# ESA-PRL/planning-path_planning

Hardware: NVIDIA B200
Metric: plans_per_s (higher is better)
Workload: dtype f64

## Files before the change

planning-path_planning_b200/build.py:

```python
import os
import subprocess
import sys

HERE = os.path.dirname(os.path.abspath(__file__))
ROOT = os.path.dirname(HERE)
INCLUDE = os.path.join(ROOT, "include")
BUILD = os.path.join(ROOT, "build")
CUDA_SO = os.path.join(HERE, "libdymu_cuda.so")
HOST_SO = os.path.join(HERE, "libdymu_b200.so")

NVCC = os.environ.get("DYMU_NVCC", "/usr/local/cuda/bin/nvcc")
CXX = os.environ.get("DYMU_CXX", "/usr/bin/g++")

NVCC_FLAGS = [
    "-gencode", "arch=compute_100a,code=sm_100a", "-lineinfo", "-O3", "-std=c++17",
    "-fmad=false", "-Xcompiler", "-fPIC", "-ccbin", CXX, "-I", INCLUDE,
]
CXX_FLAGS = ["-O2", "-std=c++14", "-fPIC", "-Wall", "-ffp-contract=off", "-I", INCLUDE,
             "-I", os.path.join(HERE, "src"), "-I", os.path.join(HERE, "shim")]


def _newer(target, sources):
    if not os.path.exists(target):
        return True
    t = os.path.getmtime(target)
    return any(os.path.getmtime(s) > t for s in sources)


def _run(cmd, verbose):
    if verbose:
        print(" ".join(cmd), flush=True)
    r = subprocess.run(cmd, stdout=subprocess.PIPE, stderr=subprocess.STDOUT, text=True)
    if r.returncode != 0:
        sys.stderr.write(r.stdout)
        raise RuntimeError("build step failed: " + " ".join(cmd[:3]) + " ...")
    if verbose and r.stdout:
        print(r.stdout)
    return r.stdout


def cuda_sources():
    d = os.path.join(HERE, "csrc")
    return sorted(os.path.join(d, f) for f in os.listdir(d) if f.endswith(".cu"))


def host_sources():
    d = os.path.join(HERE, "src")
    srcs = sorted(os.path.join(d, f) for f in os.listdir(d) if f.endswith(".cpp"))
    srcs.append(os.path.join(HERE, "capi", "planner_capi.cpp"))
    return srcs


def build_cuda(force=False, verbose=False, ptxas_v=False):
    os.makedirs(BUILD, exist_ok=True)
    headers = [os.path.join(HERE, "csrc", f) for f in os.listdir(os.path.join(HERE, "csrc"))
               if f.endswith((".cuh", ".h"))] + [os.path.join(INCLUDE, "dymu_cuda.h")]
    objs = []
    log = ""
    for src in cuda_sources():
        obj = os.path.join(BUILD, os.path.basename(src)[:-3] + ".o")
        objs.append(obj)
        if force or _newer(obj, [src] + headers):
            extra = ["-Xptxas", "-v"] if ptxas_v else []
            if os.environ.get("DYMU_FIM_PROFILE"):
                extra.append("-DDYMU_FIM_PROFILE")
            if os.environ.get("DYMU_LOCAL_PROFILE"):
                extra.append("-DDYMU_LOCAL_PROFILE")
            log += _run([NVCC] + NVCC_FLAGS + extra + ["-c", src, "-o", obj], verbose)
    if force or _newer(CUDA_SO, objs):
        _run([NVCC, "-shared", "-gencode", "arch=compute_100a,code=sm_100a", "-ccbin", CXX,
              "-o", CUDA_SO] + objs + ["-cudart", "shared"], verbose)
    return log


def build_host(force=False, verbose=False):
    srcs = host_sources()
    hdrs = [os.path.join(HERE, "src", f) for f in os.listdir(os.path.join(HERE, "src"))
            if f.endswith((".hpp", ".h"))]
    hdrs += [os.path.join(INCLUDE, f) for f in os.listdir(INCLUDE)]
    if force or _newer(HOST_SO, srcs + hdrs + [CUDA_SO]):
        _run([CXX] + CXX_FLAGS + ["-shared", "-DDYMU_CAPI_B200"] + srcs +
             ["-o", HOST_SO, "-L", HERE, "-ldymu_cuda", "-Wl,-rpath,$ORIGIN"], verbose)


def build_all(force=False, verbose=False, ptxas_v=False):
    log = build_cuda(force, verbose, ptxas_v)
    if os.path.exists(os.path.join(HERE, "src", "DyMu.hpp")):
        build_host(force, verbose)
    return log


if __name__ == "__main__":
    out = build_all(force="--force" in sys.argv, verbose="--verbose" in sys.argv,
                    ptxas_v="--ptxas" in sys.argv)
    if "--ptxas" in sys.argv:
        print(out)
    print("built", CUDA_SO, "and", HOST_SO if os.path.exists(HOST_SO) else "(host lib pending)")
```

planning-path_planning_b200/csrc/dymu_path.cu:

```cuda
#include <limits.h>

#include "dymu_ctx.cuh"

namespace
{
constexpr int PATCH = 64;
constexpr int PATCH_LEAD = 20;

struct Patch
{
    double* t;
    double* e;
    double* gx;
    double* gy;
    int x0, y0;
    bool valid;
};

struct PathArgs
{
    const double* T;
    const double* elev;
    uint32_t pitch, nx, ny;
    double gres, tau;
    double x0, y0;
    uint32_t goal_i, goal_j;
    double* out;
    uint32_t cap;
    uint32_t* result;
};

__device__ __forceinline__ double grad_axis(double f, bool has_lo, double flo, bool has_hi,
                                            double fhi)
{
    const double inf = DYMU_INF;
    if ((!has_lo && !has_hi) || (has_lo && has_hi && flo == inf && fhi == inf)) return 0;
    if (!has_lo || flo == inf)
    {
        if (!has_hi) return 0;
        return fhi - f;
    }
    if (!has_hi || fhi == inf) return f - flo;
    return (fhi - flo) * 0.5;
}

__device__ __forceinline__ void grad_node(const PathArgs& a, const Patch& pt, uint32_t i, uint32_t j,
                                          double& dnx, double& dny)
{
    const double* Tc = pt.t + ((int)j - pt.y0) * PATCH + ((int)i - pt.x0);
    double f = *Tc;
    bool hl = i > 0, hr = i + 1 < a.nx, hd = j > 0, hu = j + 1 < a.ny;
    double fl = hl ? Tc[-1] : 0, fr = hr ? Tc[1] : 0;
    double fd = hd ? Tc[-PATCH] : 0, fu = hu ? Tc[PATCH] : 0;
    double dx = grad_axis(f, hl, fl, hr, fr);
    double dy = grad_axis(f, hd, fd, hu, fu);
    if ((dx == 0) && (dy == 0))
    {
        dnx = 0;
        dny = 0;
    }
    else
    {
        double n = sqrt(dx * dx + dy * dy);
        dnx = dx / n;
        dny = dy / n;
    }
}

constexpr int PATH_THREADS = 256;

struct PatchCmd
{
    int x0, y0;
};

__device__ __forceinline__ void load_patch(const PathArgs& a, double* pt_t, double* pt_e, int x0, int y0)
{
    for (int k = threadIdx.x; k < PATCH * PATCH; k += PATH_THREADS)
    {
        int r = k / PATCH, c = k % PATCH;
        int gx = x0 + c, gy = y0 + r;
        double tv = DYMU_INF, ev = 0.0;
        if (gx >= 0 && gy >= 0 && gx < (int)a.nx && gy < (int)a.ny)
        {
            tv = __ldcg(a.T + (size_t)gy * a.pitch + gx);
            ev = a.elev[(size_t)gy * a.pitch + gx];
        }
        pt_t[k] = tv;
        pt_e[k] = ev;
    }
}

__device__ __forceinline__ void patch_gradients(const PathArgs& a, const Patch& pt)
{
    for (int k = threadIdx.x; k < PATCH * PATCH; k += PATH_THREADS)
    {
        int r = k / PATCH, c = k % PATCH;
        int gx = pt.x0 + c, gy = pt.y0 + r;
        double dnx = 0, dny = 0;
        if (r >= 1 && c >= 1 && r < PATCH - 1 && c < PATCH - 1 && gx >= 0 && gy >= 0 && gx < (int)a.nx
            && gy < (int)a.ny)
            grad_node(a, pt, (uint32_t)gx, (uint32_t)gy, dnx, dny);
        pt.gx[k] = dnx;
        pt.gy[k] = dny;
    }
}

__device__ __forceinline__ void ensure_patch(const PathArgs& a, Patch& pt, PatchCmd* cmd, int lane, int cx,
                                             int cy, double dirx, double diry)
{
    if (pt.valid && cx - 1 >= pt.x0 && cy - 1 >= pt.y0 && cx + 2 < pt.x0 + PATCH && cy + 2 < pt.y0 + PATCH)
        return;
    int lx = (dirx == dirx) ? (int)(dirx * PATCH_LEAD) : 0, ly = (diry == diry) ? (int)(diry * PATCH_LEAD) : 0;
    lx = max(-PATCH_LEAD, min(PATCH_LEAD, lx));
    ly = max(-PATCH_LEAD, min(PATCH_LEAD, ly));
    pt.x0 = cx - PATCH / 2 + lx;
    pt.y0 = cy - PATCH / 2 + ly;
    pt.valid = true;
    if (lane == 0)
    {
        cmd->x0 = pt.x0;
        cmd->y0 = pt.y0;
    }
    __syncthreads();
    load_patch(a, pt.t, pt.e, pt.x0, pt.y0);
    __syncthreads();
    patch_gradients(a, pt);
    __syncthreads();
}

template <bool UNIT_RES>
__device__ __forceinline__ bool next_waypoint(const PathArgs& a, Patch& pt, PatchCmd* cmd, int lane,
                                              double wx, double wy, double& z, double& dCx,
                                              double& dCy, double& nx_, double& ny_)
{
    double gx = UNIT_RES ? wx : wx / a.gres, gy = UNIT_RES ? wy : wy / a.gres;
    if (!(gx >= 0.0) || !(gy >= 0.0) || !(gx < (double)(a.nx - 1)) || !(gy < (double)(a.ny - 1)))
        return false;
    uint32_t cx = (uint32_t)gx, cy = (uint32_t)gy;
    double da = gx - (double)cx, db = gy - (double)cy;
    ensure_patch(a, pt, cmd, lane, (int)cx, (int)cy, -dCx, -dCy);
    const int k00 = ((int)cy - pt.y0) * PATCH + ((int)cx - pt.x0);
    const int k10 = k00 + 1, k01 = k00 + PATCH, k11 = k00 + PATCH + 1;
    const double gx00 = pt.gx[k00], gx10 = pt.gx[k10], gx01 = pt.gx[k01], gx11 = pt.gx[k11];
    const double gy00 = pt.gy[k00], gy10 = pt.gy[k10], gy01 = pt.gy[k01], gy11 = pt.gy[k11];
    const double e00 = pt.e[k00], e10 = pt.e[k10], e01 = pt.e[k01], e11 = pt.e[k11];
    dCx = dymu_interp(da, db, gx00, gx01, gx10, gx11);
    dCy = dymu_interp(da, db, gy00, gy01, gy10, gy11);
    z = dymu_interp(da, db, e00, e10, e01, e11);
    nx_ = wx - a.gres * a.tau * dCx;
    ny_ = wy - a.gres * a.tau * dCy;
    return true;
}

__device__ __forceinline__ double dist2(double ax, double ay, double bx, double by)
{
    return (ax - bx) * (ax - bx) + (ay - by) * (ay - by);
}
__device__ __forceinline__ double next_up(double x) { return __longlong_as_double(__double_as_longlong(x) + 1); }
__device__ __forceinline__ double next_down(double x) { return __longlong_as_double(__double_as_longlong(x) - 1); }
__device__ double sqrt_gt_threshold(double c)
{
    if (!(c > 0)) return (c == 0) ? 0.0 : -1.0;
    double t = c * c;
    while (sqrt(t) > c) t = next_down(t);
    while (sqrt(next_up(t)) <= c) t = next_up(t);
    return t;
}
__device__ double sqrt_lt_threshold(double c)
{
    if (!(c > 0)) return 0.0;
    double t = c * c;
    while (sqrt(t) < c) t = next_up(t);
    while (t > 0 && sqrt(next_down(t)) >= c) t = next_down(t);
    return t;
}

template <bool UNIT_RES>
__global__ void __launch_bounds__(PATH_THREADS, 1) k_global_path(const PathArgs* args_arr)
{
    const PathArgs a = args_arr[blockIdx.x];
    const int lane = threadIdx.x & 31;
    extern __shared__ __align__(16) double path_smem[];
    __shared__ PatchCmd cmd;
    Patch pt;
    pt.t = path_smem;
    pt.e = path_smem + PATCH * PATCH;
    pt.gx = path_smem + 2 * PATCH * PATCH;
    pt.gy = path_smem + 3 * PATCH * PATCH;
    pt.x0 = pt.y0 = 0;
    pt.valid = false;
    if (threadIdx.x >= 32)
    {
        for (;;)
        {
            __syncthreads();
            const int x0 = cmd.x0, y0 = cmd.y0;
            if (x0 == INT_MIN) return;
            pt.x0 = x0;
            pt.y0 = y0;
            load_patch(a, pt.t, pt.e, x0, y0);
            __syncthreads();
            patch_gradients(a, pt);
            __syncthreads();
        }
    }
    const double sx = a.gres * (double)a.goal_i, sy = a.gres * (double)a.goal_j;
    uint32_t n = 0, status = DYMU_PATH_OK;
    double wx = a.x0, wy = a.y0, z, dCx = 0, dCy = 0, nx_, ny_;

    auto push = [&](double x, double y, double zz, double dx, double dy) -> bool {
        if (n >= a.cap) return false;
        if (lane == 0)
        {
            double* o = a.out + (size_t)5 * n;
            o[0] = x; o[1] = y; o[2] = zz; o[3] = dx; o[4] = dy;
        }
        n++;
        return true;
    };

    if (!next_waypoint<UNIT_RES>(a, pt, &cmd, lane, wx, wy, z, dCx, dCy, nx_, ny_)) status = DYMU_PATH_OUTSIDE;
    else if (isnan(nx_) || isnan(ny_)) status = DYMU_PATH_NAN;
    else
    {
        push(wx, wy, z, dCx, dCy);
        wx = nx_;
        wy = ny_;
        const double far2 = sqrt_gt_threshold(2.0 * a.gres);
        const double stall2 = sqrt_lt_threshold(0.01 * a.tau * a.gres);
        while (dist2(wx, wy, sx, sy) > far2)
        {
            if (!next_waypoint<UNIT_RES>(a, pt, &cmd, lane, wx, wy, z, dCx, dCy, nx_, ny_))
            {
                status = DYMU_PATH_OUTSIDE;
                break;
            }
            if (!push(wx, wy, z, dCx, dCy))
            {
                status = DYMU_PATH_CAPACITY;
                break;
            }
            if (dist2(wx, wy, nx_, ny_) < stall2)
            {
                status = DYMU_PATH_STALLED;
                break;
            }
            wx = nx_;
            wy = ny_;
        }
    }
    if (lane == 0)
    {
        a.result[0] = n;
        a.result[1] = status;
        cmd.x0 = INT_MIN;
    }
    __syncthreads();
}

int launch_paths(dymu_ctx* ctx, uint32_t n, size_t smem, const PathArgs* d_args)
{
    auto kernel = (ctx->gres == 1.0) ? k_global_path<true> : k_global_path<false>;
    DYMU_CUDA_TRY(ctx, cudaFuncSetAttribute(kernel, cudaFuncAttributeMaxDynamicSharedMemorySize, (int)smem));
    kernel<<<n, PATH_THREADS, smem, ctx->stream>>>(d_args);
    return DYMU_OK;
}
}

extern "C" {

int dymu_extract_global_path(dymu_ctx* ctx, uint32_t slot, double x0, double y0, double tau,
                             uint32_t goal_i, uint32_t goal_j, double* out, uint32_t cap,
                             uint32_t* n_out, int* status)
{
    DYMU_GUARD(ctx);
    if (!ctx || !out || !n_out || !status || cap == 0 || slot >= ctx->n_slots) return DYMU_ERR_ARG;
    if (goal_i >= ctx->nx || goal_j >= ctx->ny) return DYMU_ERR_ARG;
    size_t out_bytes = (size_t)cap * 5 * sizeof(double);
    size_t hdr = 256;
    DYMU_TRY(dymu_internal_scratch(ctx, hdr + out_bytes, hdr + out_bytes));
    PathArgs* h_args = (PathArgs*)ctx->h_pinned;
    PathArgs a;
    a.T = ctx->T + (size_t)slot * ctx->pitch * ctx->rows;
    a.elev = ctx->elev;
    a.pitch = ctx->pitch; a.nx = ctx->nx; a.ny = ctx->ny;
    a.gres = ctx->gres; a.tau = tau; a.x0 = x0; a.y0 = y0;
    a.goal_i = goal_i; a.goal_j = goal_j;
    a.out = (double*)((char*)ctx->d_scratch + hdr);
    a.cap = cap;
    a.result = (uint32_t*)((char*)ctx->d_scratch + sizeof(PathArgs));
    static_assert(sizeof(PathArgs) + 8 <= 256, "path header overflow");
    *h_args = a;
    DYMU_CUDA_TRY(ctx, cudaMemcpyAsync(ctx->d_scratch, h_args, sizeof(PathArgs),
                                       cudaMemcpyHostToDevice, ctx->stream));
    const size_t smem = 4 * PATCH * PATCH * sizeof(double);
    DYMU_TRY(launch_paths(ctx, 1, smem, (const PathArgs*)ctx->d_scratch));
    ctx->launches++;
    DYMU_CUDA_TRY(ctx, cudaGetLastError());
    uint32_t* h_res = (uint32_t*)((char*)ctx->h_pinned + sizeof(PathArgs));
    DYMU_CUDA_TRY(ctx, cudaMemcpyAsync(h_res, a.result, 8, cudaMemcpyDeviceToHost, ctx->stream));
    DYMU_CUDA_TRY(ctx, cudaStreamSynchronize(ctx->stream));
    *n_out = h_res[0];
    *status = (int)h_res[1];
    if (h_res[0])
    {
        DYMU_CUDA_TRY(ctx, cudaMemcpyAsync(out, a.out, (size_t)h_res[0] * 5 * sizeof(double),
                                           cudaMemcpyDeviceToHost, ctx->stream));
        DYMU_CUDA_TRY(ctx, cudaStreamSynchronize(ctx->stream));
    }
    return DYMU_OK;
}

int dymu_extract_global_path_batch(dymu_ctx* ctx, uint32_t n, const uint32_t* slots,
                                   const double* xy0, double tau, const uint32_t* goal_ij,
                                   double* out, uint32_t cap, uint32_t* n_out, int* status)
{
    DYMU_GUARD(ctx);
    if (!ctx || !slots || !xy0 || !goal_ij || !out || !n_out || !status || n == 0 || cap == 0)
        return DYMU_ERR_ARG;
    for (uint32_t q = 0; q < n; ++q)
        if (slots[q] >= ctx->n_slots || goal_ij[2 * q] >= ctx->nx || goal_ij[2 * q + 1] >= ctx->ny)
            return DYMU_ERR_ARG;
    const size_t hdr = (((size_t)n * (sizeof(PathArgs) + 8)) + 255) & ~(size_t)255;
    const size_t out_bytes = (size_t)n * cap * 5 * sizeof(double);
    DYMU_TRY(dymu_internal_scratch(ctx, hdr + out_bytes, hdr));
    PathArgs* h_args = (PathArgs*)ctx->h_pinned;
    char* d_base = (char*)ctx->d_scratch;
    uint32_t* d_res = (uint32_t*)(d_base + (size_t)n * sizeof(PathArgs));
    for (uint32_t q = 0; q < n; ++q)
    {
        PathArgs a;
        a.T = ctx->T + (size_t)slots[q] * ctx->pitch * ctx->rows;
        a.elev = ctx->elev;
        a.pitch = ctx->pitch; a.nx = ctx->nx; a.ny = ctx->ny;
        a.gres = ctx->gres; a.tau = tau; a.x0 = xy0[2 * q]; a.y0 = xy0[2 * q + 1];
        a.goal_i = goal_ij[2 * q]; a.goal_j = goal_ij[2 * q + 1];
        a.out = (double*)(d_base + hdr) + (size_t)q * cap * 5;
        a.cap = cap;
        a.result = d_res + 2 * q;
        h_args[q] = a;
    }
    DYMU_CUDA_TRY(ctx, cudaMemcpyAsync(d_base, h_args, (size_t)n * sizeof(PathArgs), cudaMemcpyHostToDevice,
                                       ctx->stream));
    const size_t smem = 4 * PATCH * PATCH * sizeof(double);
    DYMU_TRY(launch_paths(ctx, n, smem, (const PathArgs*)d_base));
    ctx->launches++;
    DYMU_CUDA_TRY(ctx, cudaGetLastError());
    uint32_t* h_res = (uint32_t*)((char*)ctx->h_pinned + (size_t)n * sizeof(PathArgs));
    DYMU_CUDA_TRY(ctx, cudaMemcpyAsync(h_res, d_res, (size_t)n * 8, cudaMemcpyDeviceToHost, ctx->stream));
    DYMU_CUDA_TRY(ctx, cudaStreamSynchronize(ctx->stream));
    for (uint32_t q = 0; q < n; ++q)
    {
        n_out[q] = h_res[2 * q];
        status[q] = (int)h_res[2 * q + 1];
        if (n_out[q])
            DYMU_CUDA_TRY(ctx, cudaMemcpyAsync(out + (size_t)q * cap * 5,
                                               (double*)(d_base + hdr) + (size_t)q * cap * 5,
                                               (size_t)n_out[q] * 5 * sizeof(double), cudaMemcpyDeviceToHost,
                                               ctx->stream));
    }
    DYMU_CUDA_TRY(ctx, cudaStreamSynchronize(ctx->stream));
    return DYMU_OK;
}

}
```

Before: 99.37.

## Double-buffer prefetched gradient windows with warp-specialized helper threads in path kernel

Restructures the path-extraction kernel so one warp walks the gradient descent while the other warps build the next 64x64 window (gradients plus elevation) into a second shared-memory buffer, coordinated through named barriers. It predicts where the walk will leave the current window and prefetches there, so window building is meant to overlap with walking instead of stalling it. Gradients are now computed straight from global T, which drops the staging pass and the extra block-wide syncs. The walk step also uses clamped window indexing with an in-window flag in place of a per-step bounds check. The cost is more complex synchronization: a wrong prediction still forces a blocking rebuild, and a shutdown path with a stop flag is needed. It also adds an optional profiling build flag.

```diff
diff --git a/planning-path_planning_b200/build.py b/planning-path_planning_b200/build.py
--- a/planning-path_planning_b200/build.py
+++ b/planning-path_planning_b200/build.py
@@ -66,6 +66,8 @@
                 extra.append("-DDYMU_FIM_PROFILE")
             if os.environ.get("DYMU_LOCAL_PROFILE"):
                 extra.append("-DDYMU_LOCAL_PROFILE")
+            if os.environ.get("DYMU_PATH_PROFILE"):
+                extra.append("-DDYMU_PATH_PROFILE")
             log += _run([NVCC] + NVCC_FLAGS + extra + ["-c", src, "-o", obj], verbose)
     if force or _newer(CUDA_SO, objs):
         _run([NVCC, "-shared", "-gencode", "arch=compute_100a,code=sm_100a", "-ccbin", CXX,
diff --git a/planning-path_planning_b200/csrc/dymu_path.cu b/planning-path_planning_b200/csrc/dymu_path.cu
--- a/planning-path_planning_b200/csrc/dymu_path.cu
+++ b/planning-path_planning_b200/csrc/dymu_path.cu
@@ -1,21 +1,20 @@
 #include <limits.h>
+#include <stdio.h>
+#include <stdlib.h>
 
 #include "dymu_ctx.cuh"
 
 namespace
 {
 constexpr int PATCH = 64;
+constexpr int P2 = PATCH * PATCH;
+constexpr int WIN_DOUBLES = 3 * P2;
+constexpr size_t PATH_SMEM = 2 * WIN_DOUBLES * sizeof(double);
 constexpr int PATCH_LEAD = 20;
-
-struct Patch
-{
-    double* t;
-    double* e;
-    double* gx;
-    double* gy;
-    int x0, y0;
-    bool valid;
-};
+constexpr int PATH_THREADS = 256;
+constexpr int HELPERS = PATH_THREADS - 32;
+constexpr int BUILD_BATCH = 4;
+constexpr int BAR_CMD = 1, BAR_DONE = 2;
 
 struct PathArgs
 {
@@ -28,6 +27,9 @@
     double* out;
     uint32_t cap;
     uint32_t* result;
+#ifdef DYMU_PATH_PROFILE
+    unsigned long long* prof;
+#endif
 };
 
 __device__ __forceinline__ double grad_axis(double f, bool has_lo, double flo, bool has_hi,
@@ -44,113 +46,139 @@
     return (fhi - flo) * 0.5;
 }
 
-__device__ __forceinline__ void grad_node(const PathArgs& a, const Patch& pt, uint32_t i, uint32_t j,
-                                          double& dnx, double& dny)
-{
-    const double* Tc = pt.t + ((int)j - pt.y0) * PATCH + ((int)i - pt.x0);
-    double f = *Tc;
-    bool hl = i > 0, hr = i + 1 < a.nx, hd = j > 0, hu = j + 1 < a.ny;
-    double fl = hl ? Tc[-1] : 0, fr = hr ? Tc[1] : 0;
-    double fd = hd ? Tc[-PATCH] : 0, fu = hu ? Tc[PATCH] : 0;
-    double dx = grad_axis(f, hl, fl, hr, fr);
-    double dy = grad_axis(f, hd, fd, hu, fu);
-    if ((dx == 0) && (dy == 0))
-    {
-        dnx = 0;
-        dny = 0;
-    }
-    else
-    {
-        double n = sqrt(dx * dx + dy * dy);
-        dnx = dx / n;
-        dny = dy / n;
-    }
-}
-
-constexpr int PATH_THREADS = 256;
-
-struct PatchCmd
-{
-    int x0, y0;
+struct WinCmd
+{
+    int x0, y0, buf, stop;
 };
 
-__device__ __forceinline__ void load_patch(const PathArgs& a, double* pt_t, double* pt_e, int x0, int y0)
-{
-    for (int k = threadIdx.x; k < PATCH * PATCH; k += PATH_THREADS)
-    {
-        int r = k / PATCH, c = k % PATCH;
-        int gx = x0 + c, gy = y0 + r;
-        double tv = DYMU_INF, ev = 0.0;
-        if (gx >= 0 && gy >= 0 && gx < (int)a.nx && gy < (int)a.ny)
-        {
-            tv = __ldcg(a.T + (size_t)gy * a.pitch + gx);
-            ev = a.elev[(size_t)gy * a.pitch + gx];
-        }
-        pt_t[k] = tv;
-        pt_e[k] = ev;
-    }
-}
-
-__device__ __forceinline__ void patch_gradients(const PathArgs& a, const Patch& pt)
-{
-    for (int k = threadIdx.x; k < PATCH * PATCH; k += PATH_THREADS)
-    {
-        int r = k / PATCH, c = k % PATCH;
-        int gx = pt.x0 + c, gy = pt.y0 + r;
-        double dnx = 0, dny = 0;
-        if (r >= 1 && c >= 1 && r < PATCH - 1 && c < PATCH - 1 && gx >= 0 && gy >= 0 && gx < (int)a.nx
-            && gy < (int)a.ny)
-            grad_node(a, pt, (uint32_t)gx, (uint32_t)gy, dnx, dny);
-        pt.gx[k] = dnx;
-        pt.gy[k] = dny;
-    }
-}
-
-__device__ __forceinline__ void ensure_patch(const PathArgs& a, Patch& pt, PatchCmd* cmd, int lane, int cx,
-                                             int cy, double dirx, double diry)
-{
-    if (pt.valid && cx - 1 >= pt.x0 && cy - 1 >= pt.y0 && cx + 2 < pt.x0 + PATCH && cy + 2 < pt.y0 + PATCH)
-        return;
-    int lx = (dirx == dirx) ? (int)(dirx * PATCH_LEAD) : 0, ly = (diry == diry) ? (int)(diry * PATCH_LEAD) : 0;
-    lx = max(-PATCH_LEAD, min(PATCH_LEAD, lx));
-    ly = max(-PATCH_LEAD, min(PATCH_LEAD, ly));
-    pt.x0 = cx - PATCH / 2 + lx;
-    pt.y0 = cy - PATCH / 2 + ly;
-    pt.valid = true;
-    if (lane == 0)
-    {
-        cmd->x0 = pt.x0;
-        cmd->y0 = pt.y0;
-    }
-    __syncthreads();
-    load_patch(a, pt.t, pt.e, pt.x0, pt.y0);
-    __syncthreads();
-    patch_gradients(a, pt);
-    __syncthreads();
-}
+__device__ __forceinline__ void bar_arrive(int id)
+{
+    asm volatile("bar.arrive %0, %1;" ::"r"(id), "n"(PATH_THREADS) : "memory");
+}
+__device__ __forceinline__ void bar_sync(int id)
+{
+    asm volatile("bar.sync %0, %1;" ::"r"(id), "n"(PATH_THREADS) : "memory");
+}
+
+__device__ __forceinline__ void build_window(const PathArgs& a, double* wb, int x0, int y0,
+                                             const volatile int* stop)
+{
+    const int t = threadIdx.x - 32;
+    for (int k0 = 0; k0 < P2; k0 += BUILD_BATCH * HELPERS)
+    {
+        if (*stop) return;
+        double f[BUILD_BATCH], fl[BUILD_BATCH], fr[BUILD_BATCH], fd[BUILD_BATCH], fu[BUILD_BATCH];
+        double ev[BUILD_BATCH];
+        bool hl[BUILD_BATCH], hr[BUILD_BATCH], hd[BUILD_BATCH], hu[BUILD_BATCH], inner[BUILD_BATCH];
+#pragma unroll
+        for (int u = 0; u < BUILD_BATCH; ++u)
+        {
+            const int k = k0 + u * HELPERS + t;
+            const int r = k / PATCH, c = k % PATCH;
+            const int gx = x0 + c, gy = y0 + r;
+            const bool in_grid = k < P2 && gx >= 0 && gy >= 0 && gx < (int)a.nx && gy < (int)a.ny;
+            inner[u] = in_grid && r >= 1 && c >= 1 && r < PATCH - 1 && c < PATCH - 1;
+            hl[u] = gx > 0;
+            hr[u] = gx + 1 < (int)a.nx;
+            hd[u] = gy > 0;
+            hu[u] = gy + 1 < (int)a.ny;
+            const size_t at = in_grid ? (size_t)gy * a.pitch + gx : 0;
+            ev[u] = in_grid ? a.elev[at] : 0.0;
+            f[u] = fl[u] = fr[u] = fd[u] = fu[u] = 0;
+            if (inner[u])
+            {
+                const double* Tc = a.T + at;
+                f[u] = __ldcg(Tc);
+                if (hl[u]) fl[u] = __ldcg(Tc - 1);
+                if (hr[u]) fr[u] = __ldcg(Tc + 1);
+                if (hd[u]) fd[u] = __ldcg(Tc - a.pitch);
+                if (hu[u]) fu[u] = __ldcg(Tc + a.pitch);
+            }
+        }
+#pragma unroll
+        for (int u = 0; u < BUILD_BATCH; ++u)
+        {
+            const int k = k0 + u * HELPERS + t;
+            double dnx = 0, dny = 0;
+            if (inner[u])
+            {
+                const double dx = grad_axis(f[u], hl[u], fl[u], hr[u], fr[u]);
+                const double dy = grad_axis(f[u], hd[u], fd[u], hu[u], fu[u]);
+                if (!((dx == 0) && (dy == 0)))
+                {
+                    const double nrm = sqrt(dx * dx + dy * dy);
+                    dnx = dx / nrm;
+                    dny = dy / nrm;
+                }
+            }
+            if (k < P2)
+            {
+                wb[k] = dnx;
+                wb[P2 + k] = dny;
+                wb[2 * P2 + k] = ev[u];
+            }
+        }
+    }
+}
+
+__device__ __forceinline__ void place_window(int cx, int cy, double dirx, double diry, int& x0, int& y0)
+{
+    const double m = fmax(fabs(dirx), fabs(diry));
+    int lx = 0, ly = 0;
+    if (m > 0)
+    {
+        lx = (int)(PATCH_LEAD * (dirx / m));
+        ly = (int)(PATCH_LEAD * (diry / m));
+    }
+    x0 = cx - PATCH / 2 + lx;
+    y0 = cy - PATCH / 2 + ly;
+}
+
+__device__ __forceinline__ void predict_window(double gx, double gy, double dirx, double diry, int x0,
+                                               int y0, int& px0, int& py0)
+{
+    if (!(dirx == dirx) || !(diry == diry)) dirx = diry = 0;
+    double t = 1e30;
+    if (dirx > 0) t = fmin(t, ((double)(x0 + PATCH - 2) - gx) / dirx);
+    if (dirx < 0) t = fmin(t, (gx - (double)(x0 + 1)) / -dirx);
+    if (diry > 0) t = fmin(t, ((double)(y0 + PATCH - 2) - gy) / diry);
+    if (diry < 0) t = fmin(t, (gy - (double)(y0 + 1)) / -diry);
+    if (!(t < 1e30)) t = 0;
+    t = fmax(t, 0.0);
+    place_window((int)floor(gx + t * dirx), (int)floor(gy + t * diry), dirx, diry, px0, py0);
+}
+
+struct Step
+{
+    double z, dCx, dCy, nx, ny, gx, gy;
+    int cx, cy;
+    bool outside, inwin;
+};
 
 template <bool UNIT_RES>
-__device__ __forceinline__ bool next_waypoint(const PathArgs& a, Patch& pt, PatchCmd* cmd, int lane,
-                                              double wx, double wy, double& z, double& dCx,
-                                              double& dCy, double& nx_, double& ny_)
-{
-    double gx = UNIT_RES ? wx : wx / a.gres, gy = UNIT_RES ? wy : wy / a.gres;
-    if (!(gx >= 0.0) || !(gy >= 0.0) || !(gx < (double)(a.nx - 1)) || !(gy < (double)(a.ny - 1)))
-        return false;
-    uint32_t cx = (uint32_t)gx, cy = (uint32_t)gy;
-    double da = gx - (double)cx, db = gy - (double)cy;
-    ensure_patch(a, pt, cmd, lane, (int)cx, (int)cy, -dCx, -dCy);
-    const int k00 = ((int)cy - pt.y0) * PATCH + ((int)cx - pt.x0);
-    const int k10 = k00 + 1, k01 = k00 + PATCH, k11 = k00 + PATCH + 1;
-    const double gx00 = pt.gx[k00], gx10 = pt.gx[k10], gx01 = pt.gx[k01], gx11 = pt.gx[k11];
-    const double gy00 = pt.gy[k00], gy10 = pt.gy[k10], gy01 = pt.gy[k01], gy11 = pt.gy[k11];
-    const double e00 = pt.e[k00], e10 = pt.e[k10], e01 = pt.e[k01], e11 = pt.e[k11];
-    dCx = dymu_interp(da, db, gx00, gx01, gx10, gx11);
-    dCy = dymu_interp(da, db, gy00, gy01, gy10, gy11);
-    z = dymu_interp(da, db, e00, e10, e01, e11);
-    nx_ = wx - a.gres * a.tau * dCx;
-    ny_ = wy - a.gres * a.tau * dCy;
-    return true;
+__device__ __forceinline__ void walk_step(const PathArgs& a, const double* wb, int x0, int y0, double wx,
+                                          double wy, double c_step, double lim_x, double lim_y, Step& s)
+{
+    const double gx = UNIT_RES ? wx : wx / a.gres, gy = UNIT_RES ? wy : wy / a.gres;
+    s.gx = gx;
+    s.gy = gy;
+    s.outside = !(gx >= 0.0) || !(gy >= 0.0) || !(gx < lim_x) || !(gy < lim_y);
+    const int cx = __double2int_rz(gx), cy = __double2int_rz(gy);
+    const double da = gx - trunc(gx), db = gy - trunc(gy);
+    s.cx = cx;
+    s.cy = cy;
+    const int lx = (int)((unsigned)cx - (unsigned)x0), ly = (int)((unsigned)cy - (unsigned)y0);
+    const int kx = min(max(lx, 1), PATCH - 3), ky = min(max(ly, 1), PATCH - 3);
+    s.inwin = (kx == lx) && (ky == ly);
+    const double* g = wb + ky * PATCH + kx;
+    const double gx00 = g[0], gx10 = g[1], gx01 = g[PATCH], gx11 = g[PATCH + 1];
+    const double gy00 = g[P2], gy10 = g[P2 + 1], gy01 = g[P2 + PATCH], gy11 = g[P2 + PATCH + 1];
+    const double e00 = g[2 * P2], e10 = g[2 * P2 + 1], e01 = g[2 * P2 + PATCH], e11 = g[2 * P2 + PATCH + 1];
+    s.dCx = dymu_interp(da, db, gx00, gx01, gx10, gx11);
+    s.dCy = dymu_interp(da, db, gy00, gy01, gy10, gy11);
+    s.z = dymu_interp(da, db, e00, e10, e01, e11);
+    s.nx = wx - c_step * s.dCx;
+    s.ny = wy - c_step * s.dCy;
 }
 
 __device__ __forceinline__ double dist2(double ax, double ay, double bx, double by)
@@ -180,90 +208,155 @@
 __global__ void __launch_bounds__(PATH_THREADS, 1) k_global_path(const PathArgs* args_arr)
 {
     const PathArgs a = args_arr[blockIdx.x];
-    const int lane = threadIdx.x & 31;
     extern __shared__ __align__(16) double path_smem[];
-    __shared__ PatchCmd cmd;
-    Patch pt;
-    pt.t = path_smem;
-    pt.e = path_smem + PATCH * PATCH;
-    pt.gx = path_smem + 2 * PATCH * PATCH;
-    pt.gy = path_smem + 3 * PATCH * PATCH;
-    pt.x0 = pt.y0 = 0;
-    pt.valid = false;
+    __shared__ WinCmd cmd;
     if (threadIdx.x >= 32)
     {
         for (;;)
         {
-            __syncthreads();
-            const int x0 = cmd.x0, y0 = cmd.y0;
+            bar_sync(BAR_CMD);
+            const int x0 = cmd.x0, y0 = cmd.y0, buf = cmd.buf;
             if (x0 == INT_MIN) return;
-            pt.x0 = x0;
-            pt.y0 = y0;
-            load_patch(a, pt.t, pt.e, x0, y0);
-            __syncthreads();
-            patch_gradients(a, pt);
-            __syncthreads();
-        }
-    }
+            build_window(a, path_smem + buf * WIN_DOUBLES, x0, y0, &cmd.stop);
+            bar_arrive(BAR_DONE);
+        }
+    }
+    const int lane = threadIdx.x;
+#ifdef DYMU_PATH_PROFILE
+    const long long prof_t0 = clock64();
+    long long win_cycles = 0;
+    unsigned long long windows = 0, misses = 0;
+#define PATH_PROF(stmt) stmt
+#else
+#define PATH_PROF(stmt)
+#endif
+    auto command = [&](int buf, int x0, int y0) {
+        if (lane == 0)
+        {
+            cmd.x0 = x0;
+            cmd.y0 = y0;
+            cmd.buf = buf;
+        }
+        __syncwarp();
+        bar_arrive(BAR_CMD);
+    };
+    if (lane == 0) cmd.stop = 0;
+
     const double sx = a.gres * (double)a.goal_i, sy = a.gres * (double)a.goal_j;
+    const double c_step = a.gres * a.tau;
+    const double lim_x = (double)(a.nx - 1), lim_y = (double)(a.ny - 1);
     uint32_t n = 0, status = DYMU_PATH_OK;
-    double wx = a.x0, wy = a.y0, z, dCx = 0, dCy = 0, nx_, ny_;
-
-    auto push = [&](double x, double y, double zz, double dx, double dy) -> bool {
-        if (n >= a.cap) return false;
+    double wx = a.x0, wy = a.y0;
+    int cur = 0, x0, y0;
+    int pf_x0, pf_y0;
+    bool pending = false;
+    Step s;
+
+    auto store = [&](const Step& st, double x, double y) {
         if (lane == 0)
         {
             double* o = a.out + (size_t)5 * n;
-            o[0] = x; o[1] = y; o[2] = zz; o[3] = dx; o[4] = dy;
+            o[0] = x; o[1] = y; o[2] = st.z; o[3] = st.dCx; o[4] = st.dCy;
         }
         n++;
-        return true;
     };
 
-    if (!next_waypoint<UNIT_RES>(a, pt, &cmd, lane, wx, wy, z, dCx, dCy, nx_, ny_)) status = DYMU_PATH_OUTSIDE;
-    else if (isnan(nx_) || isnan(ny_)) status = DYMU_PATH_NAN;
+    const double g0x = UNIT_RES ? wx : wx / a.gres, g0y = UNIT_RES ? wy : wy / a.gres;
+    if (!(g0x >= 0.0) || !(g0y >= 0.0) || !(g0x < lim_x) || !(g0y < lim_y))
+        status = DYMU_PATH_OUTSIDE;
     else
     {
-        push(wx, wy, z, dCx, dCy);
-        wx = nx_;
-        wy = ny_;
-        const double far2 = sqrt_gt_threshold(2.0 * a.gres);
-        const double stall2 = sqrt_lt_threshold(0.01 * a.tau * a.gres);
-        while (dist2(wx, wy, sx, sy) > far2)
-        {
-            if (!next_waypoint<UNIT_RES>(a, pt, &cmd, lane, wx, wy, z, dCx, dCy, nx_, ny_))
+        PATH_PROF(long long t0 = clock64());
+        place_window((int)g0x, (int)g0y, 0.0, 0.0, x0, y0);
+        command(cur, x0, y0);
+        bar_sync(BAR_DONE);
+        PATH_PROF(win_cycles += clock64() - t0; windows++; misses++);
+        walk_step<UNIT_RES>(a, path_smem, x0, y0, wx, wy, c_step, lim_x, lim_y, s);
+        if (isnan(s.nx) || isnan(s.ny)) status = DYMU_PATH_NAN;
+        else
+        {
+            store(s, wx, wy);
+            predict_window(s.gx, s.gy, -s.dCx, -s.dCy, x0, y0, pf_x0, pf_y0);
+            command(cur ^ 1, pf_x0, pf_y0);
+            pending = true;
+            const double far2 = sqrt_gt_threshold(2.0 * a.gres);
+            const double stall2 = sqrt_lt_threshold(0.01 * a.tau * a.gres);
+            double px = NAN, py = NAN, dirx = -s.dCx, diry = -s.dCy;
+            wx = s.nx;
+            wy = s.ny;
+            for (;;)
             {
-                status = DYMU_PATH_OUTSIDE;
-                break;
+                walk_step<UNIT_RES>(a, path_smem + cur * WIN_DOUBLES, x0, y0, wx, wy, c_step, lim_x, lim_y, s);
+                const bool stalled = dist2(px, py, wx, wy) < stall2;
+                const bool at_goal = !(dist2(wx, wy, sx, sy) > far2);
+                const bool full = n >= a.cap;
+                if (stalled | at_goal | s.outside | !s.inwin | full)
+                {
+                    if (stalled) { status = DYMU_PATH_STALLED; break; }
+                    if (at_goal) break;
+                    if (s.outside) { status = DYMU_PATH_OUTSIDE; break; }
+                    if (!s.inwin)
+                    {
+                        PATH_PROF(long long t0 = clock64());
+                        bar_sync(BAR_DONE);
+                        const bool hit = s.cx - 1 >= pf_x0 && s.cy - 1 >= pf_y0 && s.cx + 2 < pf_x0 + PATCH
+                                         && s.cy + 2 < pf_y0 + PATCH;
+                        if (!hit)
+                        {
+                            place_window(s.cx, s.cy, dirx, diry, pf_x0, pf_y0);
+                            command(cur ^ 1, pf_x0, pf_y0);
+                            bar_sync(BAR_DONE);
+                            PATH_PROF(misses++);
+                        }
+                        cur ^= 1;
+                        x0 = pf_x0;
+                        y0 = pf_y0;
+                        predict_window(s.gx, s.gy, dirx, diry, x0, y0, pf_x0, pf_y0);
+                        command(cur ^ 1, pf_x0, pf_y0);
+                        PATH_PROF(win_cycles += clock64() - t0; windows++);
+                        continue;
+                    }
+                    status = DYMU_PATH_CAPACITY;
+                    break;
+                }
+                store(s, wx, wy);
+                px = wx;
+                py = wy;
+                dirx = -s.dCx;
+                diry = -s.dCy;
+                wx = s.nx;
+                wy = s.ny;
             }
-            if (!push(wx, wy, z, dCx, dCy))
-            {
-                status = DYMU_PATH_CAPACITY;
-                break;
-            }
-            if (dist2(wx, wy, nx_, ny_) < stall2)
-            {
-                status = DYMU_PATH_STALLED;
-                break;
-            }
-            wx = nx_;
-            wy = ny_;
-        }
-    }
+        }
+    }
+    if (pending)
+    {
+        if (lane == 0) *(volatile int*)&cmd.stop = 1;
+        __syncwarp();
+        bar_sync(BAR_DONE);
+    }
+    command(0, INT_MIN, 0);
+#ifdef DYMU_PATH_PROFILE
+    if (lane == 0 && a.prof)
+    {
+        a.prof[0] = (unsigned long long)(clock64() - prof_t0 - win_cycles);
+        a.prof[1] = (unsigned long long)win_cycles;
+        a.prof[2] = windows;
+        a.prof[3] = misses;
+    }
+#endif
     if (lane == 0)
     {
         a.result[0] = n;
         a.result[1] = status;
-        cmd.x0 = INT_MIN;
-    }
-    __syncthreads();
-}
-
-int launch_paths(dymu_ctx* ctx, uint32_t n, size_t smem, const PathArgs* d_args)
+    }
+}
+
+int launch_paths(dymu_ctx* ctx, uint32_t n, const PathArgs* d_args)
 {
     auto kernel = (ctx->gres == 1.0) ? k_global_path<true> : k_global_path<false>;
-    DYMU_CUDA_TRY(ctx, cudaFuncSetAttribute(kernel, cudaFuncAttributeMaxDynamicSharedMemorySize, (int)smem));
-    kernel<<<n, PATH_THREADS, smem, ctx->stream>>>(d_args);
+    DYMU_CUDA_TRY(ctx, cudaFuncSetAttribute(kernel, cudaFuncAttributeMaxDynamicSharedMemorySize, (int)PATH_SMEM));
+    kernel<<<n, PATH_THREADS, PATH_SMEM, ctx->stream>>>(d_args);
     return DYMU_OK;
 }
 }
@@ -290,12 +383,16 @@
     a.out = (double*)((char*)ctx->d_scratch + hdr);
     a.cap = cap;
     a.result = (uint32_t*)((char*)ctx->d_scratch + sizeof(PathArgs));
+#ifdef DYMU_PATH_PROFILE
+    a.prof = (unsigned long long*)((char*)ctx->d_scratch + sizeof(PathArgs) + 8);
+    static_assert(sizeof(PathArgs) + 8 + 4 * 8 <= 256, "path header overflow");
+#else
     static_assert(sizeof(PathArgs) + 8 <= 256, "path header overflow");
+#endif
     *h_args = a;
     DYMU_CUDA_TRY(ctx, cudaMemcpyAsync(ctx->d_scratch, h_args, sizeof(PathArgs),
                                        cudaMemcpyHostToDevice, ctx->stream));
-    const size_t smem = 4 * PATCH * PATCH * sizeof(double);
-    DYMU_TRY(launch_paths(ctx, 1, smem, (const PathArgs*)ctx->d_scratch));
+    DYMU_TRY(launch_paths(ctx, 1, (const PathArgs*)ctx->d_scratch));
     ctx->launches++;
     DYMU_CUDA_TRY(ctx, cudaGetLastError());
     uint32_t* h_res = (uint32_t*)((char*)ctx->h_pinned + sizeof(PathArgs));
@@ -303,6 +400,16 @@
     DYMU_CUDA_TRY(ctx, cudaStreamSynchronize(ctx->stream));
     *n_out = h_res[0];
     *status = (int)h_res[1];
+#ifdef DYMU_PATH_PROFILE
+    if (getenv("DYMU_TRACE_CALLS"))
+    {
+        unsigned long long* h_prof = (unsigned long long*)((char*)ctx->h_pinned + sizeof(PathArgs) + 8);
+        DYMU_CUDA_TRY(ctx, cudaMemcpyAsync(h_prof, a.prof, 4 * 8, cudaMemcpyDeviceToHost, ctx->stream));
+        DYMU_CUDA_TRY(ctx, cudaStreamSynchronize(ctx->stream));
+        fprintf(stderr, "[dymu]   path: %u waypoints, walk %llu cycles, windows %llu cycles for %llu windows "
+                "(%llu built while the walker waited)\n", h_res[0], h_prof[0], h_prof[1], h_prof[2], h_prof[3]);
+    }
+#endif
     if (h_res[0])
     {
         DYMU_CUDA_TRY(ctx, cudaMemcpyAsync(out, a.out, (size_t)h_res[0] * 5 * sizeof(double),
@@ -339,12 +446,14 @@
         a.out = (double*)(d_base + hdr) + (size_t)q * cap * 5;
         a.cap = cap;
         a.result = d_res + 2 * q;
+#ifdef DYMU_PATH_PROFILE
+        a.prof = nullptr;
+#endif
         h_args[q] = a;
     }
     DYMU_CUDA_TRY(ctx, cudaMemcpyAsync(d_base, h_args, (size_t)n * sizeof(PathArgs), cudaMemcpyHostToDevice,
                                        ctx->stream));
-    const size_t smem = 4 * PATCH * PATCH * sizeof(double);
-    DYMU_TRY(launch_paths(ctx, n, smem, (const PathArgs*)d_base));
+    DYMU_TRY(launch_paths(ctx, n, (const PathArgs*)d_base));
     ctx->launches++;
     DYMU_CUDA_TRY(ctx, cudaGetLastError());
     uint32_t* h_res = (uint32_t*)((char*)ctx->h_pinned + (size_t)n * sizeof(PathArgs));
```

After: 107.5, median of 6. +8.2%, better.
